# Wangshihu12/colmap-pcd

Hardware: AMD Instinct MI355X
Metric: NN queries/sec + BA-iter ms, 10M-pt cloud / 1M 3D feats (higher is better)
Workload: dtype f32 (NN distances) / f64 (association, BA); 1 GPU; M: 10000000-pt 'planes' cloud / 1000000 queries + BA scene 1000 cams / 1000000 pts / 4721253 obs / 900000 lidar terms (OPENCV), the same total at every N; cloud_points=10000000, queries=1000000, queries_this_rank=1000000, parallelism=single GPU

## Files before the change

### colmap-pcd_amd/csrc/cloud.h

```cpp
#pragma once
#include "common.h"

namespace pcd {

constexpr int kSortedSpare = 16;
constexpr int kBlockCells = 4;

struct GridParams {
  float origin[3];
  float h, inv_h;
  int dims[3];
  int qdims[2];
  int bdims[3];
  float slack;
};

constexpr int kMaxPyrLevels = 10;
struct PyramidParams {
  int nlev;
  int dims[kMaxPyrLevels][3];
  uint32_t off[kMaxPyrLevels];
  int seed_dims[3];
};

struct QueryScratch;

struct ShardIndex {
  uint32_t base, stride;
  uint64_t n;
  const uint32_t* g2l;
  uint64_t g2l_n;
};
__device__ __forceinline__ uint64_t shard_local_row(const ShardIndex& si, uint32_t gi) {
  if (si.g2l) {
    const uint32_t l = gi < si.g2l_n ? si.g2l[gi] : 0xFFFFFFFFu;
    return l == 0xFFFFFFFFu ? ~0ull : (uint64_t)l;
  }
  if (gi < si.base || (gi - si.base) % si.stride != 0) return ~0ull;
  const uint64_t li = (uint64_t)(gi - si.base) / si.stride;
  return li < si.n ? li : ~0ull;
}

}

struct pcd_cloud {
  int device = 0;
  uint64_t n = 0;
  uint64_t m = 0;
  uint32_t index_base = 0, index_stride = 1;
  pcd::DevBuf<uint32_t> row_index, g2l;
  uint64_t g2l_n = 0;
  pcd::DevBuf<float4> pts4, pn8, sorted;
  pcd::DevBuf<uint32_t> cell_start;
  pcd::DevBuf<float> blk_aabb;
  pcd::GridParams grid{};
  pcd::PyramidParams pyr{};
  uint64_t ncells = 0, nblocks = 0, occupied = 0;
  float bb_lo[3] = {0, 0, 0}, bb_hi[3] = {0, 0, 0};
  double build_ms = 0;
  pcd::QueryScratch* scratch = nullptr;
  pcd::ShardIndex shard_index() const { return pcd::ShardIndex{index_base, index_stride, n, g2l.p, g2l_n}; }
};

namespace pcd {
pcd_status cloud_create_indexed(const float* xyz, const float* nrm, uint64_t n, const pcd_cloud_options* opts,
                                const uint32_t* row_index, uint64_t global_n, pcd_cloud** out);
}
```

### colmap-pcd_amd/csrc/cloud.hip

```cpp
#include <cstring>

#include <rocprim/rocprim.hpp>

#include <chrono>
#include <cmath>

#include "cloud.h"
#include "grid.h"

namespace pcd {

__global__ void k_flag_rows(const float* __restrict__ xyz, const float* __restrict__ nrm, uint64_t n, int layout,
                            uint32_t* __restrict__ keep) {
  uint64_t i = blockIdx.x * (uint64_t)blockDim.x + threadIdx.x;
  if (i >= n) return;
  const float* p = layout == PCD_LAYOUT_AOS32 ? xyz + 8 * i : xyz + 3 * i;
  const float* q = layout == PCD_LAYOUT_AOS32 ? xyz + 8 * i + 4 : nrm + 3 * i;
  bool bad = isnan(p[0]) || isnan(p[1]) || isnan(p[2]) || isnan(q[0]) || isnan(q[1]) || isnan(q[2]);
  keep[i] = bad ? 0u : 1u;
}

__global__ void k_compact_rows(const float* __restrict__ xyz, const float* __restrict__ nrm, uint64_t n, int layout,
                               int raw_frame, const uint32_t* __restrict__ keep, const uint32_t* __restrict__ pos,
                               float4* __restrict__ pts4, float4* __restrict__ pn8) {
// ... 68 lines not shown
__global__ void k_cell_hist(const float4* __restrict__ pts4, uint64_t n, GridParams g, uint32_t* __restrict__ count) {
  uint64_t i = blockIdx.x * (uint64_t)blockDim.x + threadIdx.x;
  if (i >= n) return;
  float4 p = pts4[i];
  if (!(isfinite(p.x) && isfinite(p.y) && isfinite(p.z))) return;
  atomicAdd(&count[cell_of(g, p.x, p.y, p.z)], 1u);
}

__global__ void k_count_nonzero(const uint32_t* __restrict__ count, uint64_t ncells, unsigned long long* __restrict__ out) {
  unsigned c = 0;
  for (uint64_t i = blockIdx.x * (uint64_t)blockDim.x + threadIdx.x; i < ncells; i += (uint64_t)gridDim.x * blockDim.x)
    c += count[i] != 0;
  for (int off = 32; off > 0; off >>= 1) c += __shfl_xor(c, off);
  if ((threadIdx.x & 63) == 0 && c) atomicAdd(out, (unsigned long long)c);
}

__global__ void k_cell_keys(const float4* __restrict__ pts4, uint64_t n, GridParams g, uint32_t* __restrict__ keys,
                            uint32_t* __restrict__ vals) {
  uint64_t i = blockIdx.x * (uint64_t)blockDim.x + threadIdx.x;
  if (i >= n) return;
  float4 p = pts4[i];
  bool fin = isfinite(p.x) && isfinite(p.y) && isfinite(p.z);
  keys[i] = fin ? cell_of(g, p.x, p.y, p.z) : 0xFFFFFFFFu;
  vals[i] = (uint32_t)i;
}

__global__ void k_gather_sorted(const float4* __restrict__ pts4, const uint32_t* __restrict__ order, uint64_t m,
                                uint32_t index_base, uint32_t index_stride, const uint32_t* __restrict__ row_index,
                                float4* __restrict__ sorted) {
  uint64_t i = blockIdx.x * (uint64_t)blockDim.x + threadIdx.x;
  if (i >= m + kSortedSpare) return;
  uint32_t src = order[i < m ? i : m - 1];
  float4 p = pts4[src];
  p.w = __uint_as_float(row_index ? row_index[src] : index_base + src * index_stride);
  sorted[i] = p;
}

__global__ void k_leaf_aabb(const float4* __restrict__ sorted, const uint32_t* __restrict__ cell_start, GridParams g,
                            int sdx, int sdy, int sdz, float* __restrict__ aabb) {
  const int lane = threadIdx.x & 63;
  const uint64_t id = (blockIdx.x * (uint64_t)blockDim.x + threadIdx.x) >> 6;
  if (id >= (uint64_t)sdx * sdy * sdz) return;
  const int sx = (int)(id % sdx), sy = (int)((id / sdx) % sdy), sz = (int)(id / ((uint64_t)sdx * sdy));
  float lo[3] = {INFINITY, INFINITY, INFINITY}, hi[3] = {-INFINITY, -INFINITY, -INFINITY};
  const int cx0 = min(2 * sx, g.dims[0]), cx1 = min(cx0 + 2, g.dims[0]);
  const uint64_t rowbase = quad_row_base(g, sy, sz);
  const uint32_t s = cell_start[rowbase + 4 * cx0], e = cell_start[rowbase + 4 * cx1];
  for (uint32_t i = s + lane; i < e; i += 64) {
    const float4 p = sorted[i];
    lo[0] = fminf(lo[0], p.x); hi[0] = fmaxf(hi[0], p.x);
    lo[1] = fminf(lo[1], p.y); hi[1] = fmaxf(hi[1], p.y);
    lo[2] = fminf(lo[2], p.z); hi[2] = fmaxf(hi[2], p.z);
  }
  if (s != e)
    for (int off = 32; off > 0; off >>= 1)
      for (int d = 0; d < 3; ++d) {
        lo[d] = fminf(lo[d], __shfl_xor(lo[d], off));
        hi[d] = fmaxf(hi[d], __shfl_xor(hi[d], off));
      }
  if (lane == 0) {
    float* o = aabb + 8 * id;
    o[0] = lo[0]; o[1] = lo[1]; o[2] = lo[2];
    o[3] = hi[0]; o[4] = hi[1]; o[5] = hi[2];
    o[6] = __uint_as_float(s); o[7] = __uint_as_float(e - s);
  }
}

__global__ void k_pyramid_level(float* __restrict__ aabb, uint32_t off_child, int cdx, int cdy, int cdz,
                                uint32_t off_parent, int pdx, int pdy, int pdz) {
  const uint64_t id = blockIdx.x * (uint64_t)blockDim.x + threadIdx.x;
  if (id >= (uint64_t)pdx * pdy * pdz) return;
  const int px = (int)(id % pdx), py = (int)((id / pdx) % pdy), pz = (int)(id / ((uint64_t)pdx * pdy));
  float lo[3] = {INFINITY, INFINITY, INFINITY}, hi[3] = {-INFINITY, -INFINITY, -INFINITY};
  for (int k = 0; k < 4; ++k)
    for (int j = 0; j < 4; ++j)
      for (int i = 0; i < 4; ++i) {
        const int cx = 4 * px + i, cy = 4 * py + j, cz = 4 * pz + k;
        if (cx >= cdx || cy >= cdy || cz >= cdz) continue;
        const float* a = aabb + 8 * ((uint64_t)off_child + ((uint64_t)cz * cdy + cy) * cdx + cx);
        for (int d = 0; d < 3; ++d) { lo[d] = fminf(lo[d], a[d]); hi[d] = fmaxf(hi[d], a[3 + d]); }
      }
  float* o = aabb + 8 * ((uint64_t)off_parent + id);
  o[0] = lo[0]; o[1] = lo[1]; o[2] = lo[2]; o[3] = hi[0]; o[4] = hi[1]; o[5] = hi[2]; o[6] = 0.f; o[7] = 0.f;
}

static void set_dims(GridParams& g, const float lo[3], const float hi[3], float h) {
  g.h = h;
  g.inv_h = 1.0f / h;
  float ext = 0.f;
  for (int d = 0; d < 3; ++d) {
    g.origin[d] = lo[d];
    double e = (double)hi[d] - (double)lo[d];
    long c = (long)std::floor(e / h) + 1;
    if (c < 1) c = 1;
    g.dims[d] = (int)c;
    g.bdims[d] = (g.dims[d] + kBlockCells - 1) / kBlockCells;
    ext = std::fmax(ext, (float)e);
    ext = std::fmax(ext, std::fmax(std::fabs(lo[d]), std::fabs(hi[d])));
  }
  g.qdims[0] = (g.dims[1] + 1) / 2;
  g.qdims[1] = (g.dims[2] + 1) / 2;
  g.slack = ext * 9.6e-7f + 1e-30f;
}

static uint64_t num_cells(const GridParams& g) { return (uint64_t)g.dims[0] * g.qdims[0] * g.qdims[1] * 4u; }

constexpr uint64_t kMaxCells = 1ull << 26;
constexpr double kTargetOcc = 24.0;

static pcd_status build_grid(pcd_cloud* c, float user_h, hipStream_t s) {
  const uint64_t n = c->n;
  GridParams& g = c->grid;
  DevBuf<int> bb;
  DevBuf<unsigned long long> cnt;
  PCD_TRY(bb.reserve(6));
  PCD_TRY(cnt.reserve(2));
  int init[6] = {INT_MAX, INT_MAX, INT_MAX, INT_MIN, INT_MIN, INT_MIN};
  PCD_HIP_TRY(hipMemcpyAsync(bb.p, init, sizeof init, hipMemcpyHostToDevice, s));
  PCD_HIP_TRY(hipMemsetAsync(cnt.p, 0, 2 * sizeof(unsigned long long), s));
  if (n) {
    unsigned blocks = std::min<unsigned>(div_up(n, 256), 2048);
    hipLaunchKernelGGL(k_bbox, dim3(blocks), dim3(256), 0, s, c->pts4.p, n, bb.p, cnt.p);
  }
  int hb[6];
  unsigned long long hc[2];
  PCD_HIP_TRY(hipMemcpyAsync(hb, bb.p, sizeof hb, hipMemcpyDeviceToHost, s));
  PCD_HIP_TRY(hipMemcpyAsync(hc, cnt.p, sizeof hc, hipMemcpyDeviceToHost, s));
  PCD_HIP_TRY(hipStreamSynchronize(s));
  c->m = hc[0];
  float lo[3] = {0, 0, 0}, hi[3] = {0, 0, 0};
  if (c->m) for (int d = 0; d < 3; ++d) { lo[d] = ord2f(hb[d]); hi[d] = ord2f(hb[3 + d]); }
  for (int d = 0; d < 3; ++d) { c->bb_lo[d] = lo[d]; c->bb_hi[d] = hi[d]; }

  double ext[3] = {(double)hi[0] - lo[0], (double)hi[1] - lo[1], (double)hi[2] - lo[2]};
  double maxext = std::fmax(ext[0], std::fmax(ext[1], ext[2]));
  auto min_h_for_budget = [&]() {
    double h = std::cbrt((ext[0] + 1e-3) * (ext[1] + 1e-3) * (ext[2] + 1e-3) / (double)kMaxCells);
    for (int it = 0; it < 64; ++it) {
      double cells = (std::floor(ext[0] / h) + 1) * (std::floor(ext[1] / h) + 1) * (std::floor(ext[2] / h) + 1);
      if (cells <= (double)kMaxCells) break;
      h *= 1.05;
    }
    return h;
  };
  float h;
  const double hmin = std::fmax(min_h_for_budget(), 1e-6 * std::fmax(maxext, 1e-3));
  if (c->m == 0 || maxext <= 0) {
    h = user_h > 0 ? user_h : 1.0f;
  } else if (user_h > 0) {
    h = (float)std::fmax((double)user_h, hmin);
  } else {
    double hguess = std::sqrt(kTargetOcc * (ext[0] * ext[1] + ext[1] * ext[2] + ext[0] * ext[2] + 1e-6) / (double)c->m);
    h = (float)std::fmin(std::fmax(hguess, hmin), std::fmax(maxext, hmin));
    for (int it = 0; it < 6; ++it) {
      set_dims(g, lo, hi, h);
      uint64_t nc = num_cells(g);
      PCD_TRY(c->cell_start.reserve(nc + 1));
      PCD_HIP_TRY(hipMemsetAsync(c->cell_start.p, 0, (nc + 1) * sizeof(uint32_t), s));
      PCD_HIP_TRY(hipMemsetAsync(cnt.p, 0, sizeof(unsigned long long), s));
      hipLaunchKernelGGL(k_cell_hist, dim3(div_up(n, 256)), dim3(256), 0, s, c->pts4.p, n, g, c->cell_start.p);
      hipLaunchKernelGGL(k_count_nonzero, dim3(std::min<unsigned>(div_up(nc, 256), 4096)), dim3(256), 0, s,
                         c->cell_start.p, nc, cnt.p);
      PCD_HIP_TRY(hipMemcpyAsync(hc, cnt.p, sizeof(unsigned long long), hipMemcpyDeviceToHost, s));
      PCD_HIP_TRY(hipStreamSynchronize(s));
      double occ = (double)c->m / (double)std::max<unsigned long long>(hc[0], 1);
      if (occ > 0.75 * kTargetOcc && occ < 1.5 * kTargetOcc) break;
      double hn = h * std::pow(kTargetOcc / occ, 1.0 / 2.5);
      hn = std::fmin(std::fmax(hn, hmin), std::fmax(maxext, hmin));
      if (std::fabs(hn - h) < 1e-3 * h) break;
      h = (float)hn;
    }
  }
  set_dims(g, lo, hi, h);
  c->ncells = num_cells(g);
  c->nblocks = (uint64_t)g.bdims[0] * g.bdims[1] * g.bdims[2];
  if (c->ncells > kMaxCells * 2) {
    set_error("grid of %llu cells exceeds the budget", (unsigned long long)c->ncells);
    return PCD_ERR_UNSUPPORTED;
  }

  PCD_TRY(c->cell_start.reserve(c->ncells + 1));
  {
    DevBuf<uint32_t> counts;
    PCD_TRY(counts.reserve(c->ncells + 1));
    PCD_HIP_TRY(hipMemsetAsync(counts.p, 0, (c->ncells + 1) * sizeof(uint32_t), s));
    PCD_HIP_TRY(hipMemsetAsync(cnt.p, 0, sizeof(unsigned long long), s));
    if (n) hipLaunchKernelGGL(k_cell_hist, dim3(div_up(n, 256)), dim3(256), 0, s, c->pts4.p, n, g, counts.p);
    hipLaunchKernelGGL(k_count_nonzero, dim3(std::min<unsigned>(div_up(c->ncells, 256), 4096)), dim3(256), 0, s,
                       counts.p, c->ncells, cnt.p);
    PCD_HIP_TRY(hipMemcpyAsync(hc, cnt.p, sizeof(unsigned long long), hipMemcpyDeviceToHost, s));
    size_t tb = 0;
    PCD_HIP_TRY(rocprim::exclusive_scan(nullptr, tb, counts.p, c->cell_start.p, 0u, c->ncells + 1,
                                        rocprim::plus<uint32_t>(), s));
    DevBuf<char> tmp;
    PCD_TRY(tmp.reserve(tb));
    PCD_HIP_TRY(rocprim::exclusive_scan(tmp.p, tb, counts.p, c->cell_start.p, 0u, c->ncells + 1,
                                        rocprim::plus<uint32_t>(), s));
    PCD_HIP_TRY(hipStreamSynchronize(s));
  }
  c->occupied = hc[0];

  PCD_TRY(c->sorted.reserve(c->m + kSortedSpare));
  if (n) {
    DevBuf<uint32_t> k0, k1, v0, v1;
    PCD_TRY(k0.reserve(n)); PCD_TRY(k1.reserve(n)); PCD_TRY(v0.reserve(n)); PCD_TRY(v1.reserve(n));
    hipLaunchKernelGGL(k_cell_keys, dim3(div_up(n, 256)), dim3(256), 0, s, c->pts4.p, n, g, k0.p, v0.p);
    size_t tb = 0;
    PCD_HIP_TRY(rocprim::radix_sort_pairs(nullptr, tb, k0.p, k1.p, v0.p, v1.p, n, 0, 32, s));
    DevBuf<char> tmp;
    PCD_TRY(tmp.reserve(tb));
    PCD_HIP_TRY(rocprim::radix_sort_pairs(tmp.p, tb, k0.p, k1.p, v0.p, v1.p, n, 0, 32, s));
    if (c->m)
      hipLaunchKernelGGL(k_gather_sorted, dim3(div_up(c->m + kSortedSpare, 256)), dim3(256), 0, s, c->pts4.p, v1.p, c->m,
                         c->index_base, c->index_stride, c->row_index.p, c->sorted.p);
    PCD_HIP_TRY(hipStreamSynchronize(s));
  }

  PyramidParams& py = c->pyr;
  py.nlev = 1;
  py.dims[0][0] = (g.dims[0] + 1) / 2; py.dims[0][1] = g.qdims[0]; py.dims[0][2] = g.qdims[1];
  py.off[0] = 0;
  const uint64_t nleaves = (uint64_t)py.dims[0][0] * py.dims[0][1] * py.dims[0][2];
  uint64_t total_nodes = nleaves;
  while (py.nlev < kMaxPyrLevels - 1) {
    const int* pd = py.dims[py.nlev - 1];
    if ((uint64_t)pd[0] * pd[1] * pd[2] <= 64) break;
    for (int d = 0; d < 3; ++d) py.dims[py.nlev][d] = (pd[d] + 3) / 4;
    py.off[py.nlev] = (uint32_t)total_nodes;
    total_nodes += (uint64_t)py.dims[py.nlev][0] * py.dims[py.nlev][1] * py.dims[py.nlev][2];
    py.nlev++;
  }
  if ((uint64_t)py.dims[py.nlev - 1][0] * py.dims[py.nlev - 1][1] * py.dims[py.nlev - 1][2] > 64) {
    set_error("grid too large for %d pyramid levels", kMaxPyrLevels);
    return PCD_ERR_UNSUPPORTED;
  }
  for (int d = 0; d < 3; ++d) py.seed_dims[d] = (g.dims[d] + 7) / 8;
  py.dims[py.nlev][0] = py.dims[py.nlev][1] = py.dims[py.nlev][2] = 1;
  py.off[py.nlev] = (uint32_t)total_nodes;
  py.nlev++;
  PCD_TRY(c->blk_aabb.reserve(8 * total_nodes));
  hipLaunchKernelGGL(k_leaf_aabb, dim3(div_up(nleaves * 64, 256)), dim3(256), 0, s, c->sorted.p, c->cell_start.p, g,
                     py.dims[0][0], py.dims[0][1], py.dims[0][2], c->blk_aabb.p);
  for (int l = 1; l < py.nlev - 1; ++l) {
    const int* cd = py.dims[l - 1];
    const int* pd = py.dims[l];
    const uint64_t np = (uint64_t)pd[0] * pd[1] * pd[2];
    hipLaunchKernelGGL(k_pyramid_level, dim3(div_up(np, 256)), dim3(256), 0, s, c->blk_aabb.p, py.off[l - 1], cd[0],
                       cd[1], cd[2], py.off[l], pd[0], pd[1], pd[2]);
  }
  PCD_HIP_TRY(hipStreamSynchronize(s));
  PCD_HIP_TRY(hipGetLastError());
  return PCD_OK;
}

void free_query_scratch(QueryScratch* s);

}

using namespace pcd;

extern "C" {

void pcd_cloud_options_default(pcd_cloud_options* o) {
  if (!o) return;
  std::memset(o, 0, sizeof *o);
  o->layout = PCD_LAYOUT_XYZ_NRM;
  o->raw_lidar_frame = 1;
  o->index_stride = 1;
}

pcd_status pcd_cloud_create(const float* xyz, const float* nrm, uint64_t n, const pcd_cloud_options* opts,
                            pcd_cloud** out) {
  return pcd::guard([&]() -> pcd_status {
  return pcd::cloud_create_indexed(xyz, nrm, n, opts, nullptr, 0, out);
  });
}

}

__global__ static void k_fill_g2l(const uint32_t* __restrict__ row_index, uint64_t n, uint32_t* __restrict__ g2l) {
  const uint64_t i = blockIdx.x * (uint64_t)blockDim.x + threadIdx.x;
  if (i < n) g2l[row_index[i]] = (uint32_t)i;
}

pcd_status pcd::cloud_create_indexed(const float* xyz, const float* nrm, uint64_t n, const pcd_cloud_options* opts,
                                     const uint32_t* row_index, uint64_t global_n, pcd_cloud** out) {
  PCD_REQUIRE(out, "out is null");
  *out = nullptr;
  pcd_cloud_options o;
  if (opts) o = *opts; else pcd_cloud_options_default(&o);
  PCD_REQUIRE(o.layout == PCD_LAYOUT_XYZ_NRM || o.layout == PCD_LAYOUT_AOS32, "unknown layout");
  PCD_REQUIRE(n == 0 || xyz, "xyz is null");
  PCD_REQUIRE(n == 0 || o.layout == PCD_LAYOUT_AOS32 || nrm, "nrm is null");
  PCD_REQUIRE(n < 0xFFFFFFF0ull, "more than 2^32 rows");
  if (o.index_stride == 0) o.index_stride = 1;
  PCD_REQUIRE(!(o.raw_lidar_frame && (o.index_stride != 1 || o.index_base != 0)),
              "sharded clouds (index_stride/base) need raw_lidar_frame = 0");
  PCD_REQUIRE(o.cell_size >= 0 && std::isfinite(o.cell_size), "cell_size");
  PCD_TRY(require_device(o.device));

  auto t0 = std::chrono::steady_clock::now();
  pcd_cloud* c = new pcd_cloud();
  c->device = o.device;
  c->index_base = o.index_base;
  c->index_stride = o.index_stride;
  hipStream_t s = nullptr;
  auto fail = [&](pcd_status st) { pcd_cloud_destroy(c); return st; };
  if (row_index) {
    if (o.raw_lidar_frame) { set_error("indexed shards need raw_lidar_frame = 0"); return fail(PCD_ERR_INVALID); }
    pcd_status sr;
    if ((sr = c->row_index.reserve(std::max<uint64_t>(n, 1))) != PCD_OK) return fail(sr);
    if ((sr = c->g2l.reserve(std::max<uint64_t>(global_n, 1))) != PCD_OK) return fail(sr);
    c->g2l_n = global_n;
    if (n && hipMemcpy(c->row_index.p, row_index, n * sizeof(uint32_t), hipMemcpyHostToDevice) != hipSuccess) return fail(PCD_ERR_HIP);
    if (hipMemset(c->g2l.p, 0xFF, std::max<uint64_t>(global_n, 1) * sizeof(uint32_t)) != hipSuccess) return fail(PCD_ERR_HIP);
    if (n) hipLaunchKernelGGL(k_fill_g2l, dim3(div_up(n, 256)), dim3(256), 0, s, c->row_index.p, n, c->g2l.p);
  }

  const size_t row = o.layout == PCD_LAYOUT_AOS32 ? 8 : 3;
  DevBuf<float> d_xyz, d_nrm;
  DevBuf<uint32_t> keep, pos;
  pcd_status st;
  if ((st = d_xyz.reserve(std::max<size_t>(n * row, 1))) != PCD_OK) return fail(st);
  if ((st = d_nrm.reserve(std::max<size_t>(n * 3, 1))) != PCD_OK) return fail(st);
  if (n) {
    if (hipMemcpy(d_xyz.p, xyz, n * row * sizeof(float), hipMemcpyHostToDevice) != hipSuccess) return fail(PCD_ERR_HIP);
    if (o.layout == PCD_LAYOUT_XYZ_NRM &&
        hipMemcpy(d_nrm.p, nrm, n * 3 * sizeof(float), hipMemcpyHostToDevice) != hipSuccess) return fail(PCD_ERR_HIP);
  }
  uint64_t kept = n;
  if (o.raw_lidar_frame && n) {
// ... 73 lines not shown
```

### colmap-pcd_amd/csrc/nn.hip

```cpp
#include <cstring>

#include <rocprim/rocprim.hpp>

#include <atomic>
#include <cfloat>

#include "cloud.h"
#include "grid.h"
#include "scratch.h"

namespace pcd {

void free_query_scratch(QueryScratch* s) { delete s; }

constexpr uint64_t kKeyInit = (uint64_t)0x7F7FFFFFu << 32;
constexpr uint64_t kSmallBatch = 65536;

struct BrickParams {
  int B, R;
  int Bx;
  int nb[3];
  uint32_t nbricks;
};

// ... 521 lines not shown
    }
    if (threadIdx.x == 255) { s_off[nfine] = tq; s_ioff[nfine] = ti; }
    __syncthreads();
  }
  auto place = [&](const uint2 e) {
    const uint32_t f = e.x & mask, i = e.y;
    const uint32_t r = atomicAdd(&s_cur[f], 1u);
    float4 q = qf4[i];
    const uint32_t pos = beg + s_off[f] + r;
    if (r % (uint32_t)G == 0u) {
      const int cx = cell_coord_raw(q.x, g.origin[0], g.inv_h, g.dims[0]);
      const int cy = cell_coord_raw(q.y, g.origin[1], g.inv_h, g.dims[1]);
      const int cz = cell_coord_raw(q.z, g.origin[2], g.inv_h, g.dims[2]);
      const uint32_t left = s_off[f + 1] - s_off[f] - r;
      items[ibase + s_ioff[f] + r / (uint32_t)G] =
          make_uint4(pos, (uint32_t)(cx / b.Bx), (uint32_t)(cy / b.B),
                     (uint32_t)(cz / b.B) | ((left < (uint32_t)G ? left : (uint32_t)G) << 28));
    }
    q.w = __uint_as_float(i);
    qsorted[pos] = q;
    ksorted[pos] = keys_in ? keys_in[i] : kKeyInit;
  };
#pragma unroll
  for (uint32_t k = 0; k < kBkHeld; ++k)
    if (beg + threadIdx.x + k * 256u < end) place(held[k]);
  for (uint32_t p = beg + threadIdx.x + kBkHeld * 256u; p < end; p += 256) place(ppair[p]);
}

}
#include "brick_kernel.h"
#include "brick_clip_kernel.h"
namespace pcd {


constexpr uint32_t kFbcThreads = 1024, kFbcPer = 4;
__global__ __launch_bounds__(1024) void k_fb_compact(const uint32_t* __restrict__ list,
                                                     const uint32_t* __restrict__ count_ptr,
                                                     uint32_t* __restrict__ dense, uint32_t* __restrict__ dense_count) {
  __shared__ uint32_t s_wave[16], s_base;
  const uint32_t tid = threadIdx.x, lane = tid & 63, wave = tid >> 6;
  const uint32_t n = *count_ptr;
  const uint32_t e0 = (blockIdx.x * kFbcThreads + tid) * kFbcPer;
  if (blockIdx.x * kFbcThreads * kFbcPer >= n) return;
  uint32_t v[kFbcPer], cnt = 0;
  if (e0 + kFbcPer <= n) {
    const uint4 q = *reinterpret_cast<const uint4*>(list + e0);
    v[0] = q.x; v[1] = q.y; v[2] = q.z; v[3] = q.w;
  } else {
#pragma unroll
    for (uint32_t k = 0; k < kFbcPer; ++k) v[k] = e0 + k < n ? list[e0 + k] : 0xFFFFFFFFu;
  }
#pragma unroll
  for (uint32_t k = 0; k < kFbcPer; ++k) cnt += v[k] != 0xFFFFFFFFu ? 1u : 0u;
  const uint32_t inc = wave_scan_add_u32(cnt);
  if (lane == 63) s_wave[wave] = inc;
  __syncthreads();
  uint32_t before = 0, total = 0;
  for (uint32_t w = 0; w < kFbcThreads / 64; ++w) { before += w < wave ? s_wave[w] : 0u; total += s_wave[w]; }
  if (tid == 0) s_base = total ? atomicAdd(dense_count, total) : 0u;
  __syncthreads();
  uint32_t pos = s_base + before + inc - cnt;
#pragma unroll
  for (uint32_t k = 0; k < kFbcPer; ++k)
    if (v[k] != 0xFFFFFFFFu) dense[pos++] = v[k];
}

struct FbFused {
  const double* q;
  const double* max_range;
  uint64_t mr_count;
  double fixed_range;
};

template <int FUSED>
__global__ __launch_bounds__(256) void k_nn_fallback(GridParams g, PyramidParams py, const float4* __restrict__ sorted,
                                                      const uint32_t* __restrict__ cell_start,
                                                      const float* __restrict__ aabb,
                                                      const float4* __restrict__ seeds,
                                                      const float4* __restrict__ qf4,
                                                      const uint32_t* __restrict__ list,
                                                      const uint32_t* __restrict__ count_ptr, uint32_t count_imm,
                                                      uint64_t* __restrict__ keys, NnCounters* __restrict__ ctr,
                                                      int collect_stats, FbFused fu) {
  __shared__ float s_lb[4][kMaxPyrLevels][64];
  __shared__ unsigned long long s_mask[4][kMaxPyrLevels];
  __shared__ int s_node[4][kMaxPyrLevels][3];
  __shared__ int4 s_pyr[kMaxPyrLevels];
  if (threadIdx.x < (unsigned)kMaxPyrLevels)
    s_pyr[threadIdx.x] = make_int4(py.dims[threadIdx.x][0], py.dims[threadIdx.x][1], py.dims[threadIdx.x][2], (int)py.off[threadIdx.x]);
  __syncthreads();
  const int lane = threadIdx.x & 63;
  const int wave = __builtin_amdgcn_readfirstlane((int)(threadIdx.x >> 6));
  const uint32_t count = count_ptr ? *count_ptr : count_imm;
  const uint32_t nwaves = gridDim.x * 4;
  const int top = py.nlev - 1;
  const int ci = lane & 3, cj = (lane >> 2) & 3, ck = lane >> 4;
  const int tdx = py.dims[top - 1][0], tdy = py.dims[top - 1][1];
  const int tcx = lane % tdx, tcy = (lane / tdx) % tdy, tcz = lane / (tdx * tdy);
  unsigned long long st_pts = 0, st_q = 0, st_steps = 0, st_leaves = 0;
  uint32_t st_max_steps = 0, st_max_leaves = 0;
  for (uint32_t e = blockIdx.x * 4 + wave; e < count; e += nwaves) {
    const uint32_t qi = list ? list[e] : e;
    float qx, qy, qz;
    uint64_t best;
    if (FUSED == 0) {
      const float4 q = qf4[qi];
      if (q.w == 0.f) continue;
      qx = q.x; qy = q.y; qz = q.z;
      best = keys[qi];
    } else {
      qx = (float)fu.q[3 * (size_t)qi]; qy = (float)fu.q[3 * (size_t)qi + 1]; qz = (float)fu.q[3 * (size_t)qi + 2];
      if (!(isfinite(qx) && isfinite(qy) && isfinite(qz))) {
        if (lane == 0) keys[qi] = PCD_KEY_NONE;
        continue;
      }
      best = FUSED == 2 ? bounded_init_key(fu.max_range ? fu.max_range[fu.mr_count == 1 ? 0 : qi] : fu.fixed_range,
                                             fu.q[3 * (size_t)qi], fu.q[3 * (size_t)qi + 1], fu.q[3 * (size_t)qi + 2])
                          : kKeyInit;
    }
    {
      const int sx = cell_coord(qx, g.origin[0], g.inv_h, g.dims[0]) >> 3;
      const int sy = cell_coord(qy, g.origin[1], g.inv_h, g.dims[1]) >> 3;
      const int sz = cell_coord(qz, g.origin[2], g.inv_h, g.dims[2]) >> 3;
      const float4 sp = seeds[((size_t)sz * py.seed_dims[1] + sy) * py.seed_dims[0] + sx];
      const uint64_t sk = make_key(l2_simple3(qx, qy, qz, sp.x, sp.y, sp.z), __float_as_uint(sp.w));
      best = sk < best ? sk : best;
    }
    double lane_best = __builtin_bit_cast(double, best);
    float best_d = __uint_as_float((uint32_t)(best >> 32));
    int lev = top;
    int nx = 0, ny = 0, nz = 0;
    float cur_lb;
    unsigned long long cur_m;
    uint32_t rs = 0, rn = 0;
    uint32_t q_steps = 0, q_leaves = 0;
#define PCD_FB_EXPAND()                                                                                               \
    {                                                                                                                 \
      const int4 dm = s_pyr[lev - 1];                                                \
                           \
      const int cx = lev == top ? tcx : 4 * nx + ci, cy = lev == top ? tcy : 4 * ny + cj,                             \
                cz = lev == top ? tcz : 4 * nz + ck;                                                                  \
      const bool in = cx < dm.x && cy < dm.y && cz < dm.z;                                                            \
      const uint32_t id = (uint32_t)dm.w + (in ? (uint32_t)((cz * dm.y + cy) * dm.x + cx) : 0u);    \
      const float4 lo = *reinterpret_cast<const float4*>(aabb + 8 * (size_t)id);             \
      const float4 hi = *reinterpret_cast<const float4*>(aabb + 8 * (size_t)id + 4);       \
           \
                               \
      const float px = __builtin_amdgcn_fmed3f(qx, lo.x, lo.w), pyc = __builtin_amdgcn_fmed3f(qy, lo.y, hi.x),        \
                  pz = __builtin_amdgcn_fmed3f(qz, lo.z, hi.y);                                                       \
      const float lbv = l2_simple3(qx, qy, qz, px, pyc, pz);                                                          \
      cur_lb = (in && lo.x <= lo.w) ? lbv : INFINITY;                           \
      rs = __float_as_uint(hi.z); rn = __float_as_uint(hi.w);                           \
      cur_m = __ballot(cur_lb <= best_d);                                                                             \
    }
    PCD_FB_EXPAND();
    while (true) {
      ++q_steps;
      unsigned long long m = cur_m & __ballot(cur_lb <= best_d);
      if (m == 0) {
        if (lev == top) break;
        ++lev;
        cur_lb = s_lb[wave][lev][lane];
        const unsigned long long pm = s_mask[wave][lev];
        cur_m = ((unsigned long long)(uint32_t)__builtin_amdgcn_readfirstlane((int)(pm >> 32)) << 32) |
                (uint32_t)__builtin_amdgcn_readfirstlane((int)pm);
        nx = __builtin_amdgcn_readfirstlane(s_node[wave][lev][0]);
        ny = __builtin_amdgcn_readfirstlane(s_node[wave][lev][1]);
        nz = __builtin_amdgcn_readfirstlane(s_node[wave][lev][2]);
        continue;
      }
      const int sl = wave_argmin_u32(__float_as_uint(cur_lb), m);
      m &= ~(1ull << sl);
      cur_m = m;
      if (lev == 1) {
        const uint32_t s0 = (uint32_t)__builtin_amdgcn_readlane((int)rs, sl), n0 = (uint32_t)__builtin_amdgcn_readlane((int)rn, sl);
        for (uint32_t base = 0; base < n0; base += 128) {
          float4 p[2];
#pragma unroll
          for (int k = 0; k < 2; ++k) {
            const uint32_t gi = base + k * 64 + lane;
            p[k] = sorted[s0 + (gi < n0 ? gi : n0 - 1)];
          }
#pragma unroll
          for (int k = 0; k < 2; ++k) {
            const float d = l2_simple3(qx, qy, qz, p[k].x, p[k].y, p[k].z);
            lane_best = min_key_f64(lane_best, __builtin_bit_cast(double, make_key(d, __float_as_uint(p[k].w))));
          }
        }
        st_pts += n0;
        ++q_leaves;
        best = wave_min_u64(__builtin_bit_cast(uint64_t, lane_best));
        best_d = __uint_as_float((uint32_t)(best >> 32));
        unsigned long long mb = m & __ballot(cur_lb <= best_d);
        if (mb) {
          cur_m = m & ~mb;
          while (mb) {
            uint32_t a[4], c[4];
            uint32_t cmax = 0;
#pragma unroll
            for (int k = 0; k < 4; ++k) {
              const int r = mb ? __ffsll((long long)mb) - 1 : -1;
              mb &= mb - 1;
              a[k] = r >= 0 ? (uint32_t)__builtin_amdgcn_readlane((int)rs, r) : a[0];
              c[k] = r >= 0 ? (uint32_t)__builtin_amdgcn_readlane((int)rn, r) : 0u;
              cmax = c[k] > cmax ? c[k] : cmax;
              st_pts += c[k];
              q_leaves += r >= 0 ? 1 : 0;
            }
            for (uint32_t base = 0; base < cmax; base += 64) {
              float4 p[4];
              const uint32_t gi = base + lane;
#pragma unroll
              for (int k = 0; k < 4; ++k) p[k] = sorted[a[k] + (gi < c[k] ? gi : (c[k] ? c[k] - 1 : 0u))];
#pragma unroll
              for (int k = 0; k < 4; ++k) {
                const float d = l2_simple3(qx, qy, qz, p[k].x, p[k].y, p[k].z);
                lane_best = min_key_f64(lane_best, __builtin_bit_cast(double, make_key(d, __float_as_uint(p[k].w))));
              }
            }
          }
          best = wave_min_u64(__builtin_bit_cast(uint64_t, lane_best));
          best_d = __uint_as_float((uint32_t)(best >> 32));
        }
      } else {
        s_lb[wave][lev][lane] = cur_lb;
        if (lane == 0) { s_mask[wave][lev] = cur_m; s_node[wave][lev][0] = nx; s_node[wave][lev][1] = ny; s_node[wave][lev][2] = nz; }
        if (lev == top) {
          nx = __builtin_amdgcn_readlane(tcx, sl); ny = __builtin_amdgcn_readlane(tcy, sl); nz = __builtin_amdgcn_readlane(tcz, sl);
        } else {
          nx = 4 * nx + (sl & 3); ny = 4 * ny + ((sl >> 2) & 3); nz = 4 * nz + (sl >> 4);
        }
        --lev;
        PCD_FB_EXPAND();
      }
    }
#undef PCD_FB_EXPAND
    if (lane == 0) keys[qi] = finalized_key(best);
    st_q += 1;
    st_steps += q_steps; st_leaves += q_leaves;
    st_max_steps = q_steps > st_max_steps ? q_steps : st_max_steps;
    st_max_leaves = q_leaves > st_max_leaves ? q_leaves : st_max_leaves;
  }
  if (collect_stats) {
    __shared__ unsigned long long s_st[4];
    __shared__ unsigned int s_mx[2];
    if (threadIdx.x < 4) s_st[threadIdx.x] = 0;
    if (threadIdx.x < 2) s_mx[threadIdx.x] = 0;
    __syncthreads();
    if (lane == 0) {
      atomicAdd(&s_st[0], st_pts); atomicAdd(&s_st[1], st_q); atomicAdd(&s_st[2], st_steps); atomicAdd(&s_st[3], st_leaves);
      atomicMax(&s_mx[0], st_max_steps); atomicMax(&s_mx[1], st_max_leaves);
    }
    __syncthreads();
    if (threadIdx.x == 0 && s_st[1]) {
      atomicAdd(&ctr->fallback_points, s_st[0]);
      atomicAdd(&ctr->pair_evals, s_st[0]);
      atomicAdd(&ctr->fallback_queries, s_st[1]);
      atomicAdd(&ctr->fb_steps, s_st[2]); atomicAdd(&ctr->fb_leaves, s_st[3]);
      atomicMax(&ctr->fb_max_steps, s_mx[0]); atomicMax(&ctr->fb_max_leaves, s_mx[1]);
    }
  }
}

constexpr unsigned g_fb_max_blocks = 16384;
static std::atomic<int> g_collect_stats{0};
#ifdef PCD_ABLATE
static const int g_brick_blocks_per_cu = std::getenv("PCD_BRICK_BLOCKS") ? std::atoi(std::getenv("PCD_BRICK_BLOCKS")) : PCD_BRICK_MINWAVES;
#else
constexpr int g_brick_blocks_per_cu = PCD_BRICK_MINWAVES;
#endif
static std::atomic<int> g_nn_kernel{0};

static std::atomic<int> g_bk_sort{0};

static pcd_status brick_slots(pcd_cloud* c, QueryScratch* sc, const BrickParams& b, hipStream_t s) {
  if (sc->bk_slot.p && sc->bk_nslots == b.nbricks) return PCD_OK;
  PCD_TRY(sc->bk_slot.reserve((size_t)b.nbricks / 32 + 1));
  DevBuf<uint32_t> flag;
  PCD_TRY(flag.reserve((size_t)b.nbricks + 1));
  hipLaunchKernelGGL(k_brick_occupied, dim3(div_up(b.nbricks, 256)), dim3(256), 0, s, c->grid, b, c->cell_start.p, flag.p);
  hipLaunchKernelGGL(k_brick_bitmap, dim3(div_up(div_up(b.nbricks, 32), 256)), dim3(256), 0, s, flag.p, b.nbricks, sc->bk_slot.p);
  PCD_HIP_TRY(hipStreamSynchronize(s));
  sc->bk_nslots = b.nbricks;
  return PCD_OK;
}

__global__ void k_seed_init(GridParams g, int sdx, int sdy, int sdz, float4* __restrict__ seeds, float4* __restrict__ qf4,
                            uint64_t* __restrict__ keys) {
  const uint64_t i = blockIdx.x * (uint64_t)blockDim.x + threadIdx.x;
  if (i >= (uint64_t)sdx * sdy * sdz) return;
  const int x = (int)(i % sdx), y = (int)((i / sdx) % sdy), z = (int)(i / ((uint64_t)sdx * sdy));
  seeds[i] = make_float4(INFINITY, INFINITY, INFINITY, 0.f);
  const float cx = 0.5f * (float)(8 * x + min(8 * x + 8, g.dims[0])), cy = 0.5f * (float)(8 * y + min(8 * y + 8, g.dims[1])),
              cz = 0.5f * (float)(8 * z + min(8 * z + 8, g.dims[2]));
  qf4[i] = make_float4(g.origin[0] + cx * g.h, g.origin[1] + cy * g.h, g.origin[2] + cz * g.h, 1.f);
  keys[i] = kKeyInit;
}
__global__ void k_seed_gather(const uint64_t* __restrict__ keys, uint64_t n, ShardIndex si, const float4* __restrict__ pts4,
                              float4* __restrict__ seeds) {
  const uint64_t i = blockIdx.x * (uint64_t)blockDim.x + threadIdx.x;
  if (i >= n) return;
  const uint64_t k = keys[i];
  const uint64_t row = k == PCD_KEY_NONE ? ~0ull : shard_local_row(si, (uint32_t)k);
  if (row == ~0ull) return;
  const float4 p = pts4[row];
  seeds[i] = make_float4(p.x, p.y, p.z, __uint_as_float((uint32_t)k));
}
static pcd_status fb_seed_table(pcd_cloud* c, QueryScratch* sc, hipStream_t s) {
  if (sc->fb_seed_ok) return PCD_OK;
  const PyramidParams& py = c->pyr;
  const uint64_t n = (uint64_t)py.seed_dims[0] * py.seed_dims[1] * py.seed_dims[2];
  DevBuf<float4> qf4;
  DevBuf<uint64_t> keys;
  DevBuf<float4>& seeds = sc->fb_seed;
  PCD_TRY(seeds.reserve(n));
  PCD_TRY(qf4.reserve(n));
// ... 321 lines not shown
```

Baseline: 787.6 million queries/s.

## Compact AABB pyramid into occupied-only records with child ranges for NN walk

Replaces the dense per-level AABB pyramid with a compacted layout that stores only occupied nodes. Each record carries its first-child index and child count, built top-down with per-level count, scan and emit kernels. The NN fallback walk now descends through these child ranges, so it loads only occupied children and no longer does per-level coordinate arithmetic or keeps node coordinates in shared memory. The cost is extra build kernels, a host sync to size the levels, and a 26-bit record-index limit.

After: 817.0 million queries/s, median of 6. +3.7%, better.

```diff
diff --git a/colmap-pcd_amd/csrc/cloud.h b/colmap-pcd_amd/csrc/cloud.h
--- a/colmap-pcd_amd/csrc/cloud.h
+++ b/colmap-pcd_amd/csrc/cloud.h
@@ -18,10 +18,10 @@
 constexpr int kMaxPyrLevels = 10;
 struct PyramidParams {
   int nlev;
-  int dims[kMaxPyrLevels][3];
-  uint32_t off[kMaxPyrLevels];
+  uint32_t root_first, root_count;
   int seed_dims[3];
 };
+constexpr uint32_t kMaxPyrRecords = 1u << 26;
 
 struct QueryScratch;
 
diff --git a/colmap-pcd_amd/csrc/cloud.hip b/colmap-pcd_amd/csrc/cloud.hip
--- a/colmap-pcd_amd/csrc/cloud.hip
+++ b/colmap-pcd_amd/csrc/cloud.hip
@@ -174,6 +174,76 @@
       }
   float* o = aabb + 8 * ((uint64_t)off_parent + id);
   o[0] = lo[0]; o[1] = lo[1]; o[2] = lo[2]; o[3] = hi[0]; o[4] = hi[1]; o[5] = hi[2]; o[6] = 0.f; o[7] = 0.f;
+}
+
+__device__ __forceinline__ bool node_occupied(const float* __restrict__ dense, uint64_t id) {
+  return dense[8 * id] <= dense[8 * id + 3];
+}
+
+__global__ void k_count_occupied(const float* __restrict__ dense, uint64_t first, uint64_t n,
+                                 unsigned long long* __restrict__ out) {
+  unsigned c = 0;
+  for (uint64_t i = blockIdx.x * (uint64_t)blockDim.x + threadIdx.x; i < n; i += (uint64_t)gridDim.x * blockDim.x)
+    c += node_occupied(dense, first + i) ? 1u : 0u;
+  for (int off = 32; off > 0; off >>= 1) c += __shfl_xor(c, off);
+  if ((threadIdx.x & 63) == 0 && c) atomicAdd(out, (unsigned long long)c);
+}
+
+__global__ void k_top_list(const float* __restrict__ dense, uint32_t off_top, uint32_t ntop, uint32_t* __restrict__ list) {
+  const uint32_t lane = threadIdx.x;
+  const bool occ = lane < ntop && node_occupied(dense, (uint64_t)off_top + lane);
+  const unsigned long long mask = __ballot(occ);
+  if (occ) list[__popcll(mask & ((1ull << lane) - 1))] = lane;
+}
+
+__device__ __forceinline__ unsigned long long child_mask(const float* __restrict__ dense, uint32_t parent, int pdx, int pdy,
+                                                         uint32_t off_child, int cdx, int cdy, int cdz, int lane,
+                                                         uint32_t* child) {
+  const int px = (int)(parent % (uint32_t)pdx), py = (int)((parent / (uint32_t)pdx) % (uint32_t)pdy),
+            pz = (int)(parent / ((uint32_t)pdx * (uint32_t)pdy));
+  const int cx = 4 * px + (lane & 3), cy = 4 * py + ((lane >> 2) & 3), cz = 4 * pz + (lane >> 4);
+  const bool in = cx < cdx && cy < cdy && cz < cdz;
+  *child = in ? (uint32_t)(((uint64_t)cz * cdy + cy) * cdx + cx) : 0u;
+  return __ballot(in && node_occupied(dense, (uint64_t)off_child + *child));
+}
+
+__global__ void k_child_count(const float* __restrict__ dense, const uint32_t* __restrict__ list, uint32_t np, int pdx,
+                              int pdy, uint32_t off_child, int cdx, int cdy, int cdz, uint32_t* __restrict__ count) {
+  const int lane = threadIdx.x & 63;
+  const uint64_t k = (blockIdx.x * (uint64_t)blockDim.x + threadIdx.x) >> 6;
+  if (k >= np) return;
+  uint32_t child;
+  const unsigned long long mask = child_mask(dense, list[k], pdx, pdy, off_child, cdx, cdy, cdz, lane, &child);
+  if (lane == 0) count[k] = (uint32_t)__popcll(mask);
+}
+
+__global__ void k_emit_children(const float* __restrict__ dense, const uint32_t* __restrict__ list, uint32_t np,
+                                uint32_t off_parent, int pdx, int pdy, uint32_t off_child, int cdx, int cdy, int cdz,
+                                const uint32_t* __restrict__ first, uint32_t base_parent, uint32_t base_child,
+                                uint32_t* __restrict__ child_list, float* __restrict__ rec) {
+  const int lane = threadIdx.x & 63;
+  const uint64_t k = (blockIdx.x * (uint64_t)blockDim.x + threadIdx.x) >> 6;
+  if (k >= np) return;
+  const uint32_t parent = list[k];
+  uint32_t child;
+  const unsigned long long mask = child_mask(dense, parent, pdx, pdy, off_child, cdx, cdy, cdz, lane, &child);
+  const uint32_t f = first[k];
+  if ((mask >> lane) & 1) child_list[f + (uint32_t)__popcll(mask & ((1ull << lane) - 1))] = child;
+  if (lane == 0) {
+    const float* a = dense + 8 * ((uint64_t)off_parent + parent);
+    float* o = rec + 8 * ((uint64_t)base_parent + k);
+    for (int d = 0; d < 6; ++d) o[d] = a[d];
+    o[6] = __uint_as_float(base_child + f); o[7] = __uint_as_float((uint32_t)__popcll(mask));
+  }
+}
+
+__global__ void k_emit_leaves(const float4* __restrict__ dense_leaves, const uint32_t* __restrict__ list, uint32_t n,
+                              float4* __restrict__ rec) {
+  const uint64_t k = blockIdx.x * (uint64_t)blockDim.x + threadIdx.x;
+  if (k >= n) return;
+  const uint64_t src = list[k];
+  rec[2 * k] = dense_leaves[2 * src];
+  rec[2 * k + 1] = dense_leaves[2 * src + 1];
 }
 
 static void set_dims(GridParams& g, const float lo[3], const float hi[3], float h) {
@@ -309,36 +379,90 @@
   }
 
   PyramidParams& py = c->pyr;
-  py.nlev = 1;
-  py.dims[0][0] = (g.dims[0] + 1) / 2; py.dims[0][1] = g.qdims[0]; py.dims[0][2] = g.qdims[1];
-  py.off[0] = 0;
-  const uint64_t nleaves = (uint64_t)py.dims[0][0] * py.dims[0][1] * py.dims[0][2];
+  int dims[kMaxPyrLevels][3];
+  uint32_t off[kMaxPyrLevels];
+  int nreal = 1;
+  dims[0][0] = (g.dims[0] + 1) / 2; dims[0][1] = g.qdims[0]; dims[0][2] = g.qdims[1];
+  off[0] = 0;
+  const uint64_t nleaves = (uint64_t)dims[0][0] * dims[0][1] * dims[0][2];
   uint64_t total_nodes = nleaves;
-  while (py.nlev < kMaxPyrLevels - 1) {
-    const int* pd = py.dims[py.nlev - 1];
-    if ((uint64_t)pd[0] * pd[1] * pd[2] <= 64) break;
-    for (int d = 0; d < 3; ++d) py.dims[py.nlev][d] = (pd[d] + 3) / 4;
-    py.off[py.nlev] = (uint32_t)total_nodes;
-    total_nodes += (uint64_t)py.dims[py.nlev][0] * py.dims[py.nlev][1] * py.dims[py.nlev][2];
-    py.nlev++;
-  }
-  if ((uint64_t)py.dims[py.nlev - 1][0] * py.dims[py.nlev - 1][1] * py.dims[py.nlev - 1][2] > 64) {
+  auto level_nodes = [&](int l) { return (uint64_t)dims[l][0] * dims[l][1] * dims[l][2]; };
+  while (nreal < kMaxPyrLevels - 1) {
+    if (level_nodes(nreal - 1) <= 64) break;
+    for (int d = 0; d < 3; ++d) dims[nreal][d] = (dims[nreal - 1][d] + 3) / 4;
+    off[nreal] = (uint32_t)total_nodes;
+    total_nodes += level_nodes(nreal);
+    nreal++;
+  }
+  if (level_nodes(nreal - 1) > 64) {
     set_error("grid too large for %d pyramid levels", kMaxPyrLevels);
     return PCD_ERR_UNSUPPORTED;
   }
   for (int d = 0; d < 3; ++d) py.seed_dims[d] = (g.dims[d] + 7) / 8;
-  py.dims[py.nlev][0] = py.dims[py.nlev][1] = py.dims[py.nlev][2] = 1;
-  py.off[py.nlev] = (uint32_t)total_nodes;
-  py.nlev++;
-  PCD_TRY(c->blk_aabb.reserve(8 * total_nodes));
+  py.nlev = nreal + 1;
+  DevBuf<float> dense;
+  PCD_TRY(dense.reserve(8 * total_nodes));
   hipLaunchKernelGGL(k_leaf_aabb, dim3(div_up(nleaves * 64, 256)), dim3(256), 0, s, c->sorted.p, c->cell_start.p, g,
-                     py.dims[0][0], py.dims[0][1], py.dims[0][2], c->blk_aabb.p);
-  for (int l = 1; l < py.nlev - 1; ++l) {
-    const int* cd = py.dims[l - 1];
-    const int* pd = py.dims[l];
-    const uint64_t np = (uint64_t)pd[0] * pd[1] * pd[2];
-    hipLaunchKernelGGL(k_pyramid_level, dim3(div_up(np, 256)), dim3(256), 0, s, c->blk_aabb.p, py.off[l - 1], cd[0],
-                       cd[1], cd[2], py.off[l], pd[0], pd[1], pd[2]);
+                     dims[0][0], dims[0][1], dims[0][2], dense.p);
+  for (int l = 1; l < nreal; ++l) {
+    const int* cd = dims[l - 1];
+    const int* pd = dims[l];
+    hipLaunchKernelGGL(k_pyramid_level, dim3(div_up(level_nodes(l), 256)), dim3(256), 0, s, dense.p, off[l - 1], cd[0],
+                       cd[1], cd[2], off[l], pd[0], pd[1], pd[2]);
+  }
+
+  DevBuf<unsigned long long> occ;
+  unsigned long long hocc[kMaxPyrLevels] = {};
+  PCD_TRY(occ.reserve(kMaxPyrLevels));
+  PCD_HIP_TRY(hipMemsetAsync(occ.p, 0, kMaxPyrLevels * sizeof(unsigned long long), s));
+  for (int l = 0; l < nreal; ++l)
+    hipLaunchKernelGGL(k_count_occupied, dim3(std::min<unsigned>(div_up(level_nodes(l), 256), 4096)), dim3(256), 0, s,
+                       dense.p, (uint64_t)off[l], level_nodes(l), occ.p + l);
+  PCD_HIP_TRY(hipMemcpyAsync(hocc, occ.p, nreal * sizeof(unsigned long long), hipMemcpyDeviceToHost, s));
+  PCD_HIP_TRY(hipStreamSynchronize(s));
+  uint64_t base[kMaxPyrLevels], total_rec = 0, max_level = 1;
+  for (int l = nreal - 1; l >= 0; --l) {
+    base[l] = total_rec;
+    total_rec += hocc[l];
+    max_level = std::max<uint64_t>(max_level, hocc[l]);
+  }
+  if (total_rec >= kMaxPyrRecords) {
+    set_error("%llu pyramid records exceed the walk's range encoding", (unsigned long long)total_rec);
+    return PCD_ERR_UNSUPPORTED;
+  }
+  py.root_first = (uint32_t)base[nreal - 1];
+  py.root_count = (uint32_t)hocc[nreal - 1];
+  PCD_TRY(c->blk_aabb.reserve(8 * std::max<uint64_t>(total_rec, 1)));
+  if (total_rec == 0) {
+    PCD_HIP_TRY(hipMemsetAsync(c->blk_aabb.p, 0, 8 * sizeof(float), s));
+  }
+  if (total_rec) {
+    DevBuf<uint32_t> list_a, list_b, cnt, first;
+    DevBuf<char> tmp;
+    PCD_TRY(list_a.reserve(max_level)); PCD_TRY(list_b.reserve(max_level));
+    PCD_TRY(cnt.reserve(max_level)); PCD_TRY(first.reserve(max_level));
+    uint32_t* cur = list_a.p;
+    uint32_t* nxt = list_b.p;
+    hipLaunchKernelGGL(k_top_list, dim3(1), dim3(64), 0, s, dense.p, off[nreal - 1], (uint32_t)level_nodes(nreal - 1), cur);
+    for (int l = nreal - 1; l >= 1; --l) {
+      const uint32_t np = (uint32_t)hocc[l];
+      const int* cd = dims[l - 1];
+      const int* pd = dims[l];
+      hipLaunchKernelGGL(k_child_count, dim3(div_up((uint64_t)np * 64, 256)), dim3(256), 0, s, dense.p, cur, np, pd[0], pd[1],
+                         off[l - 1], cd[0], cd[1], cd[2], cnt.p);
+      size_t tb = 0;
+      PCD_HIP_TRY(rocprim::exclusive_scan(nullptr, tb, cnt.p, first.p, 0u, np, rocprim::plus<uint32_t>(), s));
+      PCD_TRY(tmp.reserve(tb));
+      PCD_HIP_TRY(rocprim::exclusive_scan(tmp.p, tb, cnt.p, first.p, 0u, np, rocprim::plus<uint32_t>(), s));
+      hipLaunchKernelGGL(k_emit_children, dim3(div_up((uint64_t)np * 64, 256)), dim3(256), 0, s, dense.p, cur, np, off[l],
+                         pd[0], pd[1], off[l - 1], cd[0], cd[1], cd[2], first.p, (uint32_t)base[l], (uint32_t)base[l - 1],
+                         nxt, c->blk_aabb.p);
+      std::swap(cur, nxt);
+    }
+    hipLaunchKernelGGL(k_emit_leaves, dim3(div_up(hocc[0], 256)), dim3(256), 0, s,
+                       reinterpret_cast<const float4*>(dense.p), cur, (uint32_t)hocc[0],
+                       reinterpret_cast<float4*>(c->blk_aabb.p + 8 * base[0]));
+    PCD_HIP_TRY(hipStreamSynchronize(s));
   }
   PCD_HIP_TRY(hipStreamSynchronize(s));
   PCD_HIP_TRY(hipGetLastError());
diff --git a/colmap-pcd_amd/csrc/nn.hip b/colmap-pcd_amd/csrc/nn.hip
--- a/colmap-pcd_amd/csrc/nn.hip
+++ b/colmap-pcd_amd/csrc/nn.hip
@@ -627,21 +627,15 @@
                                                       const uint32_t* __restrict__ count_ptr, uint32_t count_imm,
                                                       uint64_t* __restrict__ keys, NnCounters* __restrict__ ctr,
                                                       int collect_stats, FbFused fu) {
-  __shared__ float s_lb[4][kMaxPyrLevels][64];
-  __shared__ unsigned long long s_mask[4][kMaxPyrLevels];
-  __shared__ int s_node[4][kMaxPyrLevels][3];
-  __shared__ int4 s_pyr[kMaxPyrLevels];
-  if (threadIdx.x < (unsigned)kMaxPyrLevels)
-    s_pyr[threadIdx.x] = make_int4(py.dims[threadIdx.x][0], py.dims[threadIdx.x][1], py.dims[threadIdx.x][2], (int)py.off[threadIdx.x]);
-  __syncthreads();
+  constexpr int kStack = kMaxPyrLevels - 2;
+  __shared__ float s_lb[4][kStack][64];
+  __shared__ uint32_t s_rng[4][kStack][64];
+  __shared__ unsigned long long s_mask[4][kStack];
   const int lane = threadIdx.x & 63;
   const int wave = __builtin_amdgcn_readfirstlane((int)(threadIdx.x >> 6));
   const uint32_t count = count_ptr ? *count_ptr : count_imm;
   const uint32_t nwaves = gridDim.x * 4;
   const int top = py.nlev - 1;
-  const int ci = lane & 3, cj = (lane >> 2) & 3, ck = lane >> 4;
-  const int tdx = py.dims[top - 1][0], tdy = py.dims[top - 1][1];
-  const int tcx = lane % tdx, tcy = (lane / tdx) % tdy, tcz = lane / (tdx * tdy);
   unsigned long long st_pts = 0, st_q = 0, st_steps = 0, st_leaves = 0;
   uint32_t st_max_steps = 0, st_max_leaves = 0;
   for (uint32_t e = blockIdx.x * 4 + wave; e < count; e += nwaves) {
@@ -674,44 +668,39 @@
     double lane_best = __builtin_bit_cast(double, best);
     float best_d = __uint_as_float((uint32_t)(best >> 32));
     int lev = top;
-    int nx = 0, ny = 0, nz = 0;
     float cur_lb;
     unsigned long long cur_m;
     uint32_t rs = 0, rn = 0;
     uint32_t q_steps = 0, q_leaves = 0;
-#define PCD_FB_EXPAND()                                                                                               \
+#define PCD_FB_EXPAND(cf, cn)                                                                                         \
     {                                                                                                                 \
-      const int4 dm = s_pyr[lev - 1];                                                \
-                           \
-      const int cx = lev == top ? tcx : 4 * nx + ci, cy = lev == top ? tcy : 4 * ny + cj,                             \
-                cz = lev == top ? tcz : 4 * nz + ck;                                                                  \
-      const bool in = cx < dm.x && cy < dm.y && cz < dm.z;                                                            \
-      const uint32_t id = (uint32_t)dm.w + (in ? (uint32_t)((cz * dm.y + cy) * dm.x + cx) : 0u);    \
+      const uint32_t cn_ = (cn);                                                                                      \
+      const uint32_t last = cn_ ? cn_ - 1u : 0u;                   \
+      const uint32_t id = (cf) + ((uint32_t)lane < last ? (uint32_t)lane : last);                                     \
       const float4 lo = *reinterpret_cast<const float4*>(aabb + 8 * (size_t)id);             \
       const float4 hi = *reinterpret_cast<const float4*>(aabb + 8 * (size_t)id + 4);       \
            \
-                               \
+                      \
       const float px = __builtin_amdgcn_fmed3f(qx, lo.x, lo.w), pyc = __builtin_amdgcn_fmed3f(qy, lo.y, hi.x),        \
                   pz = __builtin_amdgcn_fmed3f(qz, lo.z, hi.y);                                                       \
       const float lbv = l2_simple3(qx, qy, qz, px, pyc, pz);                                                          \
-      cur_lb = (in && lo.x <= lo.w) ? lbv : INFINITY;                           \
-      rs = __float_as_uint(hi.z); rn = __float_as_uint(hi.w);                           \
+      cur_lb = (uint32_t)lane < cn_ ? lbv : INFINITY;                                                                 \
+      rs = __float_as_uint(hi.z); rn = __float_as_uint(hi.w);                                                         \
       cur_m = __ballot(cur_lb <= best_d);                                                                             \
     }
-    PCD_FB_EXPAND();
+    PCD_FB_EXPAND(py.root_first, py.root_count);
     while (true) {
       ++q_steps;
       unsigned long long m = cur_m & __ballot(cur_lb <= best_d);
       if (m == 0) {
         if (lev == top) break;
         ++lev;
-        cur_lb = s_lb[wave][lev][lane];
-        const unsigned long long pm = s_mask[wave][lev];
+        cur_lb = s_lb[wave][lev - 2][lane];
+        const uint32_t pr = s_rng[wave][lev - 2][lane];
+        rs = pr & (kMaxPyrRecords - 1u); rn = (pr >> 26) + 1u;
+        const unsigned long long pm = s_mask[wave][lev - 2];
         cur_m = ((unsigned long long)(uint32_t)__builtin_amdgcn_readfirstlane((int)(pm >> 32)) << 32) |
                 (uint32_t)__builtin_amdgcn_readfirstlane((int)pm);
-        nx = __builtin_amdgcn_readfirstlane(s_node[wave][lev][0]);
-        ny = __builtin_amdgcn_readfirstlane(s_node[wave][lev][1]);
-        nz = __builtin_amdgcn_readfirstlane(s_node[wave][lev][2]);
         continue;
       }
       const int sl = wave_argmin_u32(__float_as_uint(cur_lb), m);
@@ -768,15 +757,12 @@
           best_d = __uint_as_float((uint32_t)(best >> 32));
         }
       } else {
-        s_lb[wave][lev][lane] = cur_lb;
-        if (lane == 0) { s_mask[wave][lev] = cur_m; s_node[wave][lev][0] = nx; s_node[wave][lev][1] = ny; s_node[wave][lev][2] = nz; }
-        if (lev == top) {
-          nx = __builtin_amdgcn_readlane(tcx, sl); ny = __builtin_amdgcn_readlane(tcy, sl); nz = __builtin_amdgcn_readlane(tcz, sl);
-        } else {
-          nx = 4 * nx + (sl & 3); ny = 4 * ny + ((sl >> 2) & 3); nz = 4 * nz + (sl >> 4);
-        }
+        s_lb[wave][lev - 2][lane] = cur_lb;
+        s_rng[wave][lev - 2][lane] = rs | ((rn - 1u) << 26);
+        if (lane == 0) s_mask[wave][lev - 2] = cur_m;
+        const uint32_t cf = (uint32_t)__builtin_amdgcn_readlane((int)rs, sl), cn = (uint32_t)__builtin_amdgcn_readlane((int)rn, sl);
         --lev;
-        PCD_FB_EXPAND();
+        PCD_FB_EXPAND(cf, cn);
       }
     }
 #undef PCD_FB_EXPAND
```
